# LuchnikovI/Differentiable-quantum-circuit-cuda

Hardware: AMD Instinct MI355X
Metric: gate-applications/sec (fwd+bwd) at n qubits (higher is better)
Workload: dtype c64 (f32)

## Files before the change

differentiable-quantum-circuit-cuda_amd/csrc/qdc.hip:

```cpp
#include "qdc_circuit.hpp"
#include "qdc_primitives.hpp"
#include "qdc_spec.hpp"

namespace {
template <int R>
struct SpecCheckTwo {
  __device__ __forceinline__ void operator()(qdc::cx (&xf)[R], qdc::cx (&xb)[R], const qdc::SpecEnv& E) const {
    constexpr uint32_t z[32] = {};
    qdc::spec_xchg_imm<6, false>(xf, E, z, z);
    qdc::spec_xchg<6, false>(xb, E, z, z, z, z);
  }
};
template <int R, int TB>
struct SpecCheckOne {
  __device__ __forceinline__ void operator()(qdc::cx (&x)[R], const qdc::SpecEnv& E) const {
    constexpr uint32_t z[32] = {};
    qdc::spec_xchg_imm<TB, true>(x, E, z, z);
    qdc::spec_xchg<TB, true>(x, E, z, z, z, z);
  }
};
}
#define QDC_SPEC_CHECK(name, threads, pass)                                                       \
  __global__ __launch_bounds__(threads) void name(qdc::chunk* f, qdc::chunk* b, const qdc::fop* ops, \
                                                  const qdc::cx* mats, qdc::fgeo fg, uint32_t l0,    \
// ... 381 lines not shown
#endif
}

QDC_API size_t qdc_fusion_schedule(size_t local_qubits, int backward, size_t first_inject,
                                   const int* kinds, const unsigned char* inexact,
                                   size_t n_instr, const qdc_plan_op* plan, size_t n_plan,
                                   int lcmin, int max_ops, unsigned* item_info, size_t item_cap,
                                   unsigned* stage_len, size_t stage_cap, unsigned* op_order,
                                   size_t op_cap) {
  std::vector<qdc::Instr> ins(n_instr);
  for (size_t k = 0; k < n_instr; ++k) ins[k] = qdc::Instr{kinds[k], 0, 0};
  std::vector<uint8_t> sens(n_instr, 0);
  if (inexact)
    for (size_t k = 0; k < n_instr; ++k) sens[k] = inexact[k] ? 1 : 0;
  qdc::FusionPlanner P{ins, sens, (uint32_t)local_qubits, true, true,
                             max_ops > 0 ? (uint32_t)std::min(max_ops, qdc::FMAX_OPS)
                                         : (uint32_t)qdc::FMAX_OPS,
                             lcmin > 0 ? (uint32_t)lcmin : 3u};
  using qdc::Knob;
  P.tile2_chunks = qdc::knob_uint(Knob::TILE2_CHUNKS, P.tile2_chunks);
  P.tile1_chunks = qdc::knob_uint(Knob::TILE1_CHUNKS, P.tile1_chunks);
  P.permute = P.rq_grad = qdc::knob_int(Knob::SCHED_RQ, 0) != 0;
  P.permute = qdc::knob_int(Knob::SCHED_PERM, P.permute) != 0;
  P.mirror = qdc::knob_int(Knob::SCHED_MIRROR, P.mirror) != 0;
  P.defer_q1 = qdc::knob_int(Knob::DEFER_Q1, P.defer_q1) != 0;
  P.search = qdc::knob_int(Knob::FUSE_SEARCH, P.search) != 0;
  P.perm_low = qdc::knob_uint(Knob::RQ_PERM_LOW, P.perm_low);
  P.gamma_stage_cap = qdc::knob_int(Knob::RQ_GSTAGE, P.gamma_stage_cap) != 0;
  P.split_dens = qdc::knob_int(Knob::DENS_SPLIT, P.split_dens) != 0;
  std::vector<qdc_plan_op> pl(plan, plan + n_plan);
  const std::vector<qdc::FusionItem> items = P.fuse_items(pl, backward != 0, first_inject);
  size_t ns = 0, no = 0;
  for (size_t i = 0; i < items.size(); ++i) {
    const qdc::FusionItem& it = items[i];
    std::vector<std::vector<uint32_t>> stages;
    if (it.type == qdc::ITEM_FUSED)
      stages = P.stage_partition(it.ops, pl, backward != 0);
    else
      stages.push_back(it.ops);
// ... 344 lines not shown
```

differentiable-quantum-circuit-cuda_amd/csrc/qdc_circuit.hpp:

```cpp
#pragma once

#include <algorithm>
#include <cstring>
#include <memory>
#include <vector>

#include <rccl/rccl.h>

#include "qdc/circuit.h"
#include "qdc_device.hpp"
#include "qdc_shard.hpp"
#include "qdc_stage.hpp"
#include "qdc_fusion.hpp"
#include "qdc_spec.hpp"

namespace qdc {

struct Flat {
  const qdc_complex* data;
  std::vector<size_t> off;
  std::vector<size_t> len;
  Flat(const qdc_complex* d, const size_t* lens, size_t n) : data(d), off(n), len(n) {
    size_t o = 0;
    for (size_t i = 0; i < n; ++i) {
// ... 151 lines not shown
  uint32_t n = 0;
  uint32_t g = 0;
  uint32_t nl = 0;
  uint32_t gap_bits = 0;
  uint64_t gm = 0;
  std::vector<std::unique_ptr<DevRes>> devs;
  Exchange ex;
  std::vector<Shard> sh;
  QubitMap layout;
  size_t dens_cap = 0, grads_cap = 0;
  cx* host_out = nullptr;
  size_t host_cap = 0;
  std::vector<Instr> ins;
  struct Knobs {
    int fuse = 1;
    uint32_t fuse_max_ops = FMAX_OPS;
    uint32_t fuse_lcmin = 3;
    int fuse_meas = 1;
    int use_rq = 1;
    int rq_stats = 0;
    RqKnobs rqk;
    int rq64 = 1;
    int rq_order = 2;
    int spec_mode = 1;
    uint32_t spec_min_qubits = 22;
    uint32_t spec_max = 160;
    int spec_fwd = 1;
    int spec_async = sizeof(real) == 4 ? 1 : 0;
    int rq_permute = 1;
    int rq_perm_shard = 1;
    int rq_grad32 = 1;
    int rq_maxcl = 1;
    uint32_t rq_perm_low = 0;
    int rq_gstage = 1;
    uint32_t tile1_chunks = FusionPlanner::TILE_CHUNKS_1;
    int diag_inject = 1;
    int early_inject = 1;
    int dens1_kernel = 1;
    int dens_split = 1;
    int mirror = 1;
    int spec_half = 1;
    int defer_q1 = 1;
    int fuse_search = 1;
    uint32_t fused_blocks = 0;
    int sched_cache_on = 1;
    int state_ilv = 1;
// ... 5 lines not shown
      f(Knob::FUSE_MAX_OPS, k.fuse_max_ops, 1, FMAX_OPS);
      f(Knob::FUSE_MEAS, k.fuse_meas);
      f(Knob::FUSE_LCMIN, k.fuse_lcmin, 1, LOWBITS);
      f(Knob::FUSED_BLOCKS, k.fused_blocks, 1, (int)NBMAX);
      f(Knob::RQ, k.use_rq);
      f(Knob::RQ64, k.rq64);
      f(Knob::RQ_STATS, k.rq_stats);
      f(Knob::RW, k.rqk.rq_wave);
      f(Knob::RQ_PF, k.rqk.rq_prefetch);
      f(Knob::RQ_SLOTS5, k.rqk.rq_slots5);
      f(Knob::RQ_ORDER, k.rq_order);
      f(Knob::RQ_PERM, k.rq_permute);
      f(Knob::RQ_PERM_SHARD, k.rq_perm_shard);
      f(Knob::RQ_PERM_LOW, k.rq_perm_low);
      f(Knob::RQ_GRAD32, k.rq_grad32);
      f(Knob::RQ_MAXCL, k.rq_maxcl);
      f(Knob::RQ_GSTAGE, k.rq_gstage);
      f(Knob::TILE1_CHUNKS, k.tile1_chunks);
      f(Knob::DIAG_INJECT, k.diag_inject);
      f(Knob::EARLY_INJECT, k.early_inject);
      f(Knob::DENS1, k.dens1_kernel);
      f(Knob::DENS_SPLIT, k.dens_split);
      f(Knob::MIRROR, k.mirror);
      f(Knob::DEFER_Q1, k.defer_q1);
      f(Knob::FUSE_SEARCH, k.fuse_search);
      f(Knob::SCHED_CACHE, k.sched_cache_on);
      f(Knob::SPEC, k.spec_mode);
      f(Knob::SPEC_MIN_QUBITS, k.spec_min_qubits);
      f(Knob::SPEC_MAX, k.spec_max);
      f(Knob::SPEC_FWD, k.spec_fwd);
// ... 522 lines not shown
    c.first_inject = first_injection(pl);
    return true;
  }
  size_t first_injection(const std::vector<qdc_plan_op>& pl) const {
    for (size_t i = 0; i < pl.size(); ++i)
      if (pl[i].type == QDC_PLAN_OP && is_diff_density(ins[pl[i].instr].kind)) return i;
    return pl.size();
  }
  static constexpr uint32_t TILE_CHUNKS_1 = FusionPlanner::TILE_CHUNKS_1;
  static constexpr uint32_t TILE_CHUNKS_2 = FusionPlanner::TILE_CHUNKS_2;
  FusionPlanner planner(bool mirror_fwd) const {
    FusionPlanner P{ins, inexact, nl, k.fuse != 0, k.fuse_meas != 0, k.fuse_max_ops, k.fuse_lcmin};
    P.permute = k.rq_permute && k.use_rq && (g == 0 || k.rq_perm_shard) && sizeof(real) == 4;
    P.ng = g;
    P.rq_grad = k.rq_grad32 && k.use_rq && (sizeof(real) == 4 || k.rq64);
    if (k.rq_perm_low) P.perm_low = k.rq_perm_low;
    P.tile1_chunks = k.tile1_chunks;
    P.mirror = mirror_on() && mirror_fwd;
    P.defer_q1 = k.defer_q1 != 0;
    P.search = k.fuse_search != 0;
    P.gamma_stage_cap = k.rq_gstage != 0;
    P.split_dens = k.dens_split != 0;
    return P;
  }
  void fuse_items(Call& c) const {
    c.items.clear();
    for (FusionItem& f : c.P.fuse_items(c.plan, c.backward, c.first_inject)) {
      Item it;
      static_cast<FusionItem&>(it) = std::move(f);
      if (it.type == ITEM_FUSED) it.stages = c.P.stage_partition(it.ops, c.plan, c.backward);
// ... 553 lines not shown
    auto kern = k_dens1<TB, NT>;
    QDC_TRY(fused_grid((const void*)kern, nullptr, NT, use.grid));
    fgeo g = fg;
    QDC_TRY(size_grid(ctx, g, use, false, "density"));
    return ctx.launch_block(name, bytes, kern, use.grid, (uint32_t)NT, (const chunk*)f, fops, g,
                            partials, stride);
  }
  const char* launch_rq(Ctx& ctx, const char* name, double bytes, const fgeo& fg, bool two,
                        uint32_t tbits, const RqVariant* V, uint32_t l0, chunk* f, chunk* b,
                        const fop* fops, const cx* mats, cx* partials, uint64_t stride,
                        hipFunction_t spec, GridUse& use) {
    if (!V || V->two != two || V->tbits != tbits || (spec && !V->prefix))
      return fail("internal: a register-resident pass without its kernel variant");
    if (!two && fg.ngrad > 0)
      return fail("internal: a one-state register-resident pass with %u reductions", fg.ngrad);
    QDC_TRY(fused_grid((const void*)V->kernel, spec && V->own_grid ? spec : nullptr, (int)V->threads,
                       use.grid));
    fgeo g = fg;
    QDC_TRY(size_grid(ctx, g, use, V->dyn, "fused"));
    if (spec)
      return ctx.launch_module(name, bytes, spec, use.grid, V->threads, f, b, fops, mats, g, l0,
                               partials, stride);
    return ctx.launch_block(name, bytes, V->kernel, use.grid, V->threads, f, b, fops, mats, g, l0,
                            partials, stride);
  }
  const char* fused_grid(const void* kernel, hipFunction_t fn, int nt, uint32_t& grid) {
    if (k.fused_blocks) {
      grid = k.fused_blocks;
      return nullptr;
    }
    const void* key = fn ? (const void*)fn : kernel;
    for (auto& e : fused_resident_cache)
      if (e.first == key) {
        grid = e.second;
        return nullptr;
      }
    int per_cu = 0, dev = 0, cus = 0;
    if (fn)
// ... 409 lines not shown
```

differentiable-quantum-circuit-cuda_amd/csrc/qdc_fusion.hpp:

```cpp
#pragma once

#include <stdint.h>

#include <algorithm>
#include <vector>

#include "qdc/circuit.h"
#include "qdc_kernels.hpp"
#include "qdc_knobs.hpp"
#include "qdc_rq.hpp"
#include "qdc_shard.hpp"

namespace qdc {

struct Instr {
  int kind;
  uint32_t a;
  uint32_t b;
};

inline bool is_q1_gate(int k) {
  return k == QDC_CONST_Q1 || k == QDC_CONST_Q1_NONU || k == QDC_VAR_Q1 || k == QDC_VAR_Q1_NONU;
}
inline bool is_q2_dense(int k) {
// ... 22 lines not shown
inline bool is_q1_density(int k) { return k == QDC_Q1_DENSITY || k == QDC_DIFF_Q1_DENSITY; }
inline int gate_len(int k) { return is_q2_dense(k) ? 16 : 4; }

enum ItemType : int {
  ITEM_OP = 0,
  ITEM_REMAP = 1,
  ITEM_FUSED = 2,
  ITEM_DIAG_INJECT = 3,
};
struct FusionItem {
  int type;
  std::vector<uint32_t> ops;
  uint32_t lc = 0, h = 0, hb[FMAX_ROWS] = {};
  std::vector<std::pair<uint32_t, uint32_t>> swaps;
};

struct FusionPlanner {
  static constexpr uint32_t TILE_CHUNKS_1 = 2048;
  static constexpr uint32_t TILE_CHUNKS_2 = 1024;
  const std::vector<Instr>& ins;
  const std::vector<uint8_t>& inexact;
  uint32_t nl;
  bool fuse;
  bool fuse_meas;
  uint32_t fuse_max_ops;
  uint32_t fuse_lcmin;
  uint32_t tile2_chunks = TILE_CHUNKS_2;
  uint32_t tile1_chunks = TILE_CHUNKS_1;
  bool permute = false;
  bool rq_grad = false;
  bool gamma_stage_cap = true;
  uint32_t perm_low = (uint32_t)LV + 3;
  uint32_t ng = 0;
  bool mirror = false;
  bool defer_q1 = true;
  bool split_dens = true;
  bool search = true;

  static uint32_t log2_of(uint64_t x) {
    uint32_t k = 0;
    while ((1ull << k) < x) ++k;
    return k;
  }

  uint64_t chunk_bits_of(uint32_t p) const { return p >= (uint32_t)LV ? 1ull << (p - LV) : 0ull; }
// ... 159 lines not shown
        ++i;
        continue;
      }
      if (!on || !fusable(i)) {
        items.push_back(FusionItem{ITEM_OP, {(uint32_t)i}});
        ++i;
        continue;
      }
      size_t j = i;
      while (j < plan.size() && plan[j].type == QDC_PLAN_OP && fusable(j) &&
             !(backward && j == first_inject && j > i) && !(j == msplit && j > i))
        ++j;
      const bool two = (backward && i >= first_inject) || mfwd;
      const bool gstage = two && rq_grad && gamma_stage_cap;
      const uint32_t gmax = gstage ? fuse_max_ops
                            : (two && rq_grad) ? (uint32_t)FMAX_GRAD_RQ : (uint32_t)FMAX_GRAD;
      const PassRules rules{backward, mfwd, two, gstage, gmax, T};
      std::vector<uint32_t> rem;
      for (size_t k = i; k < j; ++k) rem.push_back((uint32_t)k);
      while (!rem.empty()) {
        ScannedPass sp = search ? search_pass(plan, rem, rules)
                                : scan_pass(plan, rem.data(), rem.size(), rules, ~0ull, false);
        if (sp.ops.size() == 1) {
          items.push_back(FusionItem{ITEM_OP, sp.ops});
        } else {
          FusionItem it{ITEM_FUSED, sp.ops};
          tile_config(sp.mask, T, it.lc, it.h, it.hb);
          bool gates_only = it.lc >= NLOW - LV;
          for (uint32_t k : sp.ops) gates_only = gates_only && is_gate_op(plan[k]);
          if (permute && gates_only) permute_after(it, plan, sp.rest, j);
          items.push_back(it);
// ... 42 lines not shown
          (q & blocked) ||
          (mfwd && meas && ndens + 1 > (uint32_t)FMAX_GRAD) ||
          (conflicts_of(cls) & left) || pass.size() >= fuse_max_ops ||
          nred + isred > r.gmax || !tile_fits(mask | op_bits(g), r.T)) {
        blocked |= q;
        left |= cls;
        rest.push_back(k);
        continue;
      }
      pass.push_back(k);
      mask |= op_bits(g);
      nred += isred;
      ndens += (mfwd && meas) ? 1u : 0u;
      kind = (int)meas;
    }
    if (r.gstage && nred > (uint32_t)FMAX_GRAD_RQ) {
      bool cut = false;
      while (pass.size() > 1 && gamma_stages(pass, plan, !mfwd) > (uint32_t)FMAX_GRAD_RQ) {
        rest.push_back(pass.back());
        pass.pop_back();
        cut = true;
      }
      if (cut) std::sort(rest.begin(), rest.end());
    }
    if (defer_q1) defer_trailing_q1(pass, rest, plan, backward, per_qubit);
    for (uint32_t k : pass) sp.mask |= op_bits(plan[k]);
    return sp;
  }

  static constexpr size_t SEARCH_SEEDS = 8;
  static constexpr size_t SEARCH_WINDOW = 512;

  uint64_t tile_positions(uint64_t pos, uint32_t T) const {
// ... 1 lines not shown
    if (!tile_config(pos >> LV, T, lc, h, hb)) return 0;
    uint64_t a = (1ull << (LV + lc)) - 1;
    for (uint32_t r = 0; r < h; ++r) a |= 1ull << (LV + hb[r]);
    return a;
  }
  static uint64_t pos_bits(const qdc_plan_op& g) { return (1ull << g.pos2) | (1ull << g.pos1); }

  ScannedPass search_pass(const std::vector<qdc_plan_op>& plan, const std::vector<uint32_t>& rem,
                          const PassRules& r) const {
    ScannedPass base = scan_pass(plan, rem.data(), rem.size(), r, ~0ull, false);
    const size_t nw = std::min(rem.size(), SEARCH_WINDOW);
    auto stages_of = [&](const ScannedPass& p) {
      return (uint32_t)stage_partition(p.ops, plan, r.backward).size();
    };
    auto at_cap = [&](const ScannedPass& p, uint32_t st) {
      return p.ops.size() >= fuse_max_ops || (r.gstage && st >= (uint32_t)FMAX_GRAD_RQ) ||
             p.rest.empty();
    };
    auto width = [&](const ScannedPass& p) {
      uint64_t q = (1ull << NLOW) - 1;
      for (uint32_t k : p.ops) q |= pos_bits(plan[k]);
      return (uint32_t)__builtin_popcountll(q);
    };
    const uint32_t base_st = stages_of(base);
    if (at_cap(base, base_st) || nw < 3) return base;

    struct Cand {
      uint64_t tile;
      ScannedPass p;
      uint32_t st;
    };
// ... 482 lines not shown
```

differentiable-quantum-circuit-cuda_amd/csrc/qdc_jit.hpp:

```cpp
#pragma once

#include <dirent.h>
#include <dlfcn.h>
#include <fcntl.h>
#include <spawn.h>
#include <sys/file.h>
#include <sys/stat.h>
#include <sys/wait.h>
#include <unistd.h>

#include <algorithm>
#include <atomic>
#include <chrono>
#include <cerrno>
#include <condition_variable>
#include <csignal>
#include <cstdlib>
#include <deque>
#include <ctime>
#include <cstdio>
#include <cstring>
#include <map>
#include <mutex>
#include <set>
// ... 16 lines not shown

inline bool spec_imm() {
  static const bool on = knob_int(Knob::SPEC_IMM, 0) != 0;
  return on;
}
struct SpecStep {
  bool relayout;
  RqLayout Lc, Ln;
  fop F;
};
struct SpecKind {
  bool two;
  uint32_t tb, ns;
  bool bar;
  const char* prefix;
  const char* pass;
  uint32_t threads;
  const char* waves;
  bool half = false;
};
inline SpecKind spec_kind(const RqVariant& V, bool half = false) {
  uint32_t tb = 0;
  while ((1u << tb) < V.threads) ++tb;
  return {V.two, tb, V.ns, V.threads > 64, V.prefix, half ? V.pass_half : V.pass, V.threads,
          half ? V.waves_half : V.waves, half};
}
inline int spec_kept_slot(const RqLayout& Lc, const RqLayout& Ln) {
  if (Lc.ns != Ln.ns) return -1;
  for (uint32_t s = 0; s < Lc.ns; ++s)
    if (Lc.slot[s] == Ln.slot[s] && Lc.slot[s] != ~0u) return (int)s;
  return -1;
}
inline bool spec_half_ok(const std::vector<SpecStep>& steps) {
  bool any = false;
  for (const SpecStep& s : steps)
    if (s.relayout) {
      any = true;
      if (spec_kept_slot(s.Lc, s.Ln) < 0) return false;
    }
  return any;
// ... 191 lines not shown
           (int)QDC_RW_WAVES, (int)QDC_RW_WAVES_ONE, (int)QDC_RQ_ABL, (int)QDC_RQ_GSPLIT,
           (int)QDC_NT_LOAD, (int)QDC_NT_STORE, (int)QDC_RW_WAVES_HALF_ONE, (int)QDC_PK_ASM, (int)QDC_PK_VASM, (int)QDC_MATVEC_N,
           sizeof(real) == 8 ? " -DQDC_F64" : "");
  return b;
}
inline const char* spec_cflags() { return "--genco -O3 -std=c++17 --offload-arch=gfx950"; }
inline uint64_t spec_fingerprint(const std::string& defines, const std::string& compiler,
                                 uint64_t source_fp) {
  uint64_t h = 1469598103934665603ull;
  const std::string s = defines + "\n" + compiler + "\n" + spec_cflags() + "\n";
  h = fnv_more(h, s.data(), s.size());
  return fnv_more(h, &source_fp, sizeof source_fp);
}
inline std::string spec_kernel_name_fp(const std::string& body, const SpecKind& K, uint64_t fp) {
  char nm[48];
  uint64_t h = spec_hash(std::string(K.pass) + "\n" + body);
  h = fnv_more(h, &fp, sizeof fp);
  snprintf(nm, sizeof nm, "%s%016llx", K.prefix, (unsigned long long)h);
  return nm;
}

#ifndef QDC_SRC_FP
#define QDC_SRC_FP 0ull
#endif

struct JitObjHeader {
  char magic[8];
  uint64_t fp, name_hash, size, body_hash;
};
static_assert(sizeof(JitObjHeader) == 40, "code-object header layout");
constexpr char JIT_MAGIC[8] = {'Q', 'D', 'C', 'J', 'I', 'T', '2', '\0'};
// ... 577 lines not shown
```

differentiable-quantum-circuit-cuda_amd/csrc/qdc_kernels.hpp:

```cpp
#pragma once

#include <cstddef>

#include <hip/hip_runtime.h>
#include <stdint.h>

#include <type_traits>

namespace qdc {

#ifdef QDC_F64
using real = double;
typedef double vec16 __attribute__((ext_vector_type(2)));
#else
using real = float;
typedef float vec16 __attribute__((ext_vector_type(4)));
#endif

struct cx {
  real x, y;
};

constexpr int VEC = 16 / (int)sizeof(cx);
constexpr int LV = (VEC == 2) ? 1 : 0;
// ... 881 lines not shown
#pragma unroll
    for (int k = 0; k < RED; ++k) acc[k] = cadd(acc[k], q[k]);
  }
  __shared__ cx out[RED];
  block_reduce_store<RED>(acc, out);
  __syncthreads();
  if (threadIdx.x < RED) {
    cx* d = tab.dst[blockIdx.x] + threadIdx.x;
    *d = accumulate ? cadd(*d, out[threadIdx.x]) : out[threadIdx.x];
  }
}
#endif


#ifndef QDC_FMAX_OPS
#define QDC_FMAX_OPS 32
#endif
constexpr int FMAX_OPS = QDC_FMAX_OPS;
constexpr int FMAX_GRAD = 16;
#ifndef QDC_FMAX_GRAD_RQ
#define QDC_FMAX_GRAD_RQ 16
#endif
constexpr int FMAX_GRAD_RQ = QDC_FMAX_GRAD_RQ;
static_assert(FMAX_GRAD_RQ >= 1 && FMAX_GRAD >= 1, "at least one reduction accumulator");
static_assert(FMAX_OPS <= 64, "rq_plan keeps stage sets in 64-bit masks");
constexpr int FMAX_ROWS = 8;
constexpr int FACC = 32;

struct fop {
  uint32_t kind;
  uint32_t t1;
  uint32_t t2;
  uint32_t mat;
};

struct fgeo {
  uint64_t ntiles;
  uint32_t tpb;
  uint32_t lc;
// ... 854 lines not shown
```

differentiable-quantum-circuit-cuda_amd/csrc/qdc_knobs.hpp:

```cpp
#pragma once

#include <stdint.h>

#include <algorithm>
#include <climits>
#include <cstdio>
#include <cstdlib>
#include <string>

namespace qdc {

enum class KnobScope { Process, Context, Circuit, Call, Hook };

#define QDC_KNOBS(X)                                                                               \
                                                        \
  X(DYN, Context, "35",                                                                            \
    "static share (% of the fair share) of a dynamic-tail pass; 100: static only")                 \
  X(DYN_GRAN, Context, "1",                                                                        \
    "smallest granule (tiles per grab, a power of two <= 32) of a reducing dynamic tail")          \
  X(EVENT_FENCE, Context, "0",                                                                     \
    "1: the profiler's HIP events are default events (system-scope fence per record)")             \
  X(GRID_CAP, Context, "1048576", "grid cap of the single-gate streaming kernels")                 \
  X(RED_CAP, Context, "2048", "grid of the single-gate reduction kernels (<= 4096)")               \
  X(REV_RED, Context, "4096",                                                                      \
// ... 12 lines not shown
  X(DIAG_RU, Context, "16",                                                                        \
    "chunks per state in flight per thread of the diagonal reverse kernels")                       \
  X(DIAG_Q, Context, "1", "0: diagonal reverse launches on k_diag instead of k_diag_q")            \
  X(DIAG_RED, Context, "4096", "grid of the diagonal reverse's reducing launches (<= 4096)")       \
  X(TILE_PF, Context, "1", "0: tile-family blocks of several tiles do not prefetch the next tile") \
  X(LANE_BLK, Context, "1",                                                                        \
    "0: far-target streaming LANE launches stay on the wave variant, not k_lane_blk")              \
  X(LANE_TILE_BITS, Context, "0x8800000",                                                          \
    "mask of target byte strides 2^b whose one-state q1 applications run on the tile family")      \
  X(LANE_NOBLK_BITS, Context, "0x808000",                                                          \
    "mask of target byte strides 2^b whose far LANE applications run on the wave variant")         \
  X(LANE_U, Context, "8,1,4",                                                                      \
    "units in flight per wave of LANE launches, \"u0,u1,u2\" per op class as QDC_LANE")            \
                                                   \
  X(FUSE, Circuit, "1", "0: one HBM pass per gate (single-gate kernels only)")                     \
  X(FUSE_MAX_OPS, Circuit, "32", "gates per fused pass (1 .. FMAX_OPS)")                           \
  X(FUSE_MEAS, Circuit, "1", "0: densities / cotangent injections stay single passes")             \
  X(FUSE_LCMIN, Circuit, "3", "minimum contiguous chunk bits of a fused tile (1 .. 6)")            \
  X(FUSED_BLOCKS, Circuit, "0",                                                                    \
    "grid of fused passes (1 .. 4096); 0: as many blocks as are resident")                         \
  X(RQ, Circuit, "1", "0: gate passes on the LDS-tile kernel, not the register-resident ones")     \
  X(RQ64, Circuit, "1", "0: f64 gate passes stay on the LDS-tile kernel")                          \
  X(RQ_STATS, Circuit, "0",                                                                        \
    "1: print each register-resident pass's counts to stderr; 2: its stages too")                  \
  X(RW, Circuit, "1", "register-resident kernel choice, a bit mask (qdc_variant.hpp)")             \
  X(RQ_PF, Circuit, "1", "0: one-state register-resident passes do not prefetch the next tile")    \
  X(RQ_SLOTS5, Circuit, "1", "0: f32 one-wave passes plan four register slots, not five")          \
  X(RQ_ORDER, Circuit, "2",                                                                        \
    "register-resident tile order: 0 block-contiguous, 1 grid-strided, 2 XCD-aware")               \
  X(RQ_PERM, Circuit, "1", "0: gate-only passes keep the qubit layout (no in-store permutation)")  \
  X(RQ_PERM_SHARD, Circuit, "1", "0: no permuting passes on sharded circuits")                     \
  X(RQ_PERM_LOW, Circuit, "0", "low positions a permuting pass fills; 0: the planner's default")   \
  X(RQ_GRAD32, Circuit, "1",                                                                       \
    "0: two-state passes hold FMAX_GRAD instead of FMAX_GRAD_RQ Gamma stages")                     \
  X(RQ_MAXCL, Circuit, "1", "0: relayouts chosen greedily instead of by max closure")              \
  X(RQ_GSTAGE, Circuit, "1",                                                                       \
    "0: two-state passes capped by variable gates instead of Gamma stages")                        \
  X(TILE1_CHUNKS, Circuit, "2048", "one-state fused tile in chunks: 2048 or 1024")                 \
  X(DIAG_INJECT, Circuit, "1",                                                                     \
    "0: runs of diagonal cotangent injections stay fused injection passes")                        \
  X(EARLY_INJECT, Circuit, "1",                                                                    \
    "0: the backward's leading diagonal injection waits for its program")                          \
  X(DENS1, Circuit, "1", "0: read-only one-qubit density passes on k_fused instead of k_dens1")    \
  X(DENS_SPLIT, Circuit, "1", "0: a forward pass may hold gates and densities together")           \
  X(MIRROR, Circuit, "1",                                                                          \
    "mirrored reverse sweeps; 0: the backward schedules itself; 2: failing to mirror is an "       \
    "error")                                                                                       \
  X(DEFER_Q1, Circuit, "1", "0: trailing one-qubit stages of a pass stay there")                   \
  X(FUSE_SEARCH, Circuit, "1",                                                                     \
// ... 30 lines not shown
  X(QK_WIDE, Call, "k >= 4: 1, else 0",                                                            \
    "dense k-qubit kernel: doubled batches per wave iteration")                                    \
  X(QK_PF, Call, "k = 3: 2, k = 5: 1, else 0",                                                     \
    "dense k-qubit kernel: 1 software-pipelined batches, 2 doubled too")                           \
  X(QK_GRID, Call, "4096", "block cap of the dense k-qubit kernels' grids")                        \
  X(QK_LDS, Call, "k = 3: 2, else 1",                                                              \
    "low targets from which a dense gate runs as LDS-staged tiles; 0: never")                      \
  X(QKL_VAR, Call, "1", "k_qkl variant: 0 not pipelined, 1 pipelined, 2 half the tiles at k = 5")  \
  X(QKG_GRID, Call, "resident blocks", "block cap of the dense gradient / density kernel")         \
  X(PAULI_GRID, Call, "per kernel", "block cap of the Pauli-sum kernels")                          \
                                                     \
  X(SCHED_RQ, Hook, "0",                                                                           \
    "qdc_fusion_schedule: permuting passes and the register-resident Gamma cap")                   \
  X(SCHED_PERM, Hook, "as QDC_SCHED_RQ", "qdc_fusion_schedule: permuting passes alone")            \
  X(SCHED_MIRROR, Hook, "0", "qdc_fusion_schedule: the mirrored forward schedule")                 \
  X(TILE2_CHUNKS, Hook, "1024", "qdc_fusion_schedule: two-state fused tile in chunks")             \
  X(RQ_KEEP, Hook, "0", "qdc_rq_plan: every relayout keeps a register slot (half buffers)")        \
  X(PRECOMPILE_DUMP, Hook, "unset",                                                                \
    "qdc_precompile: directory that receives each kernel's source")                                \
  X(PRECOMPILE_COUNT, Hook, "0", "qdc_precompile: 1 counts the kernels without compiling them")

enum class Knob : int {
#define QDC_KNOB_ID(id, scope, dflt, effect) id,
  QDC_KNOBS(QDC_KNOB_ID)
#undef QDC_KNOB_ID
};

struct KnobRow {
  const char* name;
  KnobScope scope;
// ... 72 lines not shown
```

differentiable-quantum-circuit-cuda_amd/csrc/qdc_rq.hpp:

```cpp
#pragma once

#include <type_traits>

#include "qdc_kernels.hpp"

namespace qdc {

#ifndef QDC_RQ_GSPLIT
#define QDC_RQ_GSPLIT 0
#endif
#ifndef QDC_MATVEC_N
#define QDC_MATVEC_N 1
#endif

constexpr int RQ_R = 16;
constexpr uint32_t FK_RELAYOUT = 7;
constexpr int RQ_NT_ONE = 256;
constexpr int RQ_NT_TWO = 128;

struct rq_layout {
  uint32_t rp[2 * RQ_R];
  uint32_t tv[8];
};
static_assert(sizeof(rq_layout) == 160 && sizeof(rq_layout) % sizeof(cx) == 0,
// ... 358 lines not shown
               : "+{a[64:67]}"(v[16]), "+{a[68:71]}"(v[17]), "+{a[72:75]}"(v[18]), "+{a[76:79]}"(v[19]), "+{a[80:83]}"(v[20]), "+{a[84:87]}"(v[21]), "+{a[88:91]}"(v[22]), "+{a[92:95]}"(v[23]), "+{a[96:99]}"(v[24]), "+{a[100:103]}"(v[25]), "+{a[104:107]}"(v[26]), "+{a[108:111]}"(v[27]), "+{a[112:115]}"(v[28]), "+{a[116:119]}"(v[29]), "+{a[120:123]}"(v[30]), "+{a[124:127]}"(v[31])
               :
               : "memory");
}

#ifndef QDC_RQ_PF_WAVES
#define QDC_RQ_PF_WAVES 2
#endif
struct SpecEnv {
  const cx* mats;
  const fop* ops;
  real (*accw)[FACC];
  uint32_t t;
  char* bufb;
};
template <bool TWO, int NT, bool PF, class PROG = void>
__device__ __forceinline__ void rq_pass(chunk* __restrict__ f, chunk* __restrict__ b,
                                        const fop* __restrict__ ops, const cx* __restrict__ mats,
                                        fgeo fg, uint32_t l0, cx* __restrict__ partials,
                                        uint64_t slot_stride) {
  constexpr int LOGNT = NT == 64 ? 6 : NT == 128 ? 7 : NT == 256 ? 8 : 9;
  constexpr int CPT = RQ_R / VEC;
  constexpr int TA = NT * RQ_R;
  __shared__ cx buf[TA];
  __shared__ real accw[TWO ? NT / 64 : 1][TWO ? FMAX_GRAD_RQ : 1][FACC];
  const uint32_t t = threadIdx.x;
  const int wave = __builtin_amdgcn_readfirstlane((int)(t >> 6));
  if constexpr (TWO) {
    for (uint32_t i = t; i < (NT / 64) * FMAX_GRAD_RQ * FACC; i += NT) (&accw[0][0][0])[i] = 0;
    __syncthreads();
  }
  const rq_layout* L0 = reinterpret_cast<const rq_layout*>(mats + l0);
  const rqio* io = reinterpret_cast<const rqio*>(mats + l0 + sizeof(rq_layout) / sizeof(cx));
  uint64_t thr_ld = 0, thr_st = 0;
#pragma unroll
  for (int k = 0; k < LOGNT; ++k) {
    if ((t >> k) & 1u) {
      thr_ld += io->gv_ld[k];
      thr_st += io->gv_st[k];
    }
  }
  const bool gstride = fg.order == 1;
  const uint64_t tile0 = gstride ? (uint64_t)blockIdx.x
                                 : (uint64_t)xcd_block(blockIdx.x, gridDim.x, fg.order == 2) * fg.tpb;
// ... 167 lines not shown
      }
      if (!more) break;
    }
  }
  if constexpr (TWO) {
    __syncthreads();
    for (uint32_t i = t; i < fg.ngrad * FACC; i += NT) {
      const uint32_t k = i / FACC, e = i % FACC;
      real s = 0;
#pragma unroll
      for (int w = 0; w < NT / 64; ++w) s += accw[w][k][e];
      reinterpret_cast<real*>(partials + (uint64_t)k * slot_stride + (uint64_t)blockIdx.x * RED)[e] = s;
    }
  }
}
template <bool TWO, int NT, bool PF>
__global__ __launch_bounds__(NT) __attribute__((amdgpu_waves_per_eu(PF ? QDC_RQ_PF_WAVES : 4)))
void k_rq(chunk* __restrict__ f, chunk* __restrict__ b, const fop* __restrict__ ops,
          const cx* __restrict__ mats, fgeo fg, uint32_t l0, cx* __restrict__ partials,
          uint64_t slot_stride) {
  static_assert(TWO ? (NT == 128 && !PF) : (NT == 128 || NT == 256), "k_rq: not a launched variant");
  rq_pass<TWO, NT, PF>(f, b, ops, mats, fg, l0, partials, slot_stride);
}

#ifndef QDC_RW_WAVES
#define QDC_RW_WAVES 2
#endif
#ifndef QDC_RW_WAVES_HALF_ONE
#define QDC_RW_WAVES_HALF_ONE 5
#endif
#ifndef QDC_RW_WAVES_ONE
#define QDC_RW_WAVES_ONE 2
#endif
template <bool TWO, int NE, bool PF, int W, bool S5 = false, class PROG = void, bool HALF = false>
__device__ __forceinline__ void rw_pass(chunk* __restrict__ f, chunk* __restrict__ b,
                                        const fop* __restrict__ ops, const cx* __restrict__ mats,
                                        fgeo fg, uint32_t l0, cx* __restrict__ partials,
                                        uint64_t slot_stride) {
  static_assert(NE == 1 || NE == 2 || NE == 4, "k_rw: 1, 2 or 4 register groups");
  static_assert(!S5 || (NE == 2 && VEC == 2 && W == 1 && (!PF || !TWO)),
                "five slots: f32 one-wave tiles (two-state ones without prefetch)");
  static_assert(W == 1 || (W == 2 && !TWO), "k_rw: two-state tiles are one wave");
  constexpr int LOGNE = NE == 1 ? 0 : NE == 2 ? 1 : 2;
  constexpr int TB = W == 1 ? 6 : 7;
  constexpr int R = RQ_R * NE;
  constexpr int CPT = R / VEC;
  constexpr int CPG = RQ_R / VEC;
  static_assert(!HALF || (W == 1 && !std::is_void<PROG>::value), "half buffers: one-wave programs");
  __shared__ cx buf[64 * W * R / (HALF ? 2 : 1)];
  __shared__ real accw[TWO ? FMAX_GRAD_RQ : 1][FACC];
  const uint32_t lane = threadIdx.x;
  if constexpr (TWO) {
    for (uint32_t i = lane; i < FMAX_GRAD_RQ * FACC; i += 64) (&accw[0][0])[i] = 0;
  }
  const rqio* io = reinterpret_cast<const rqio*>(mats + l0 + sizeof(rq_layout) / sizeof(cx));
  uint64_t thr_ld = 0, thr_st = 0;
#pragma unroll
  for (int k = 0; k < TB; ++k) {
    if ((lane >> k) & 1u) {
      thr_ld += io->gv_ld[k];
      thr_st += io->gv_st[k];
    }
  }
  const bool gstride = fg.order == 1;
  const uint64_t tile0 = gstride ? (uint64_t)blockIdx.x
                                 : (uint64_t)xcd_block(blockIdx.x, gridDim.x, fg.order == 2) * fg.tpb;
  const uint64_t tstep = gstride ? (uint64_t)gridDim.x : 1u;
  const uint64_t nst = (QDC_DYN_TAIL && fg_arg()->ndyn) ? fg_arg()->nstat : fg.ntiles;
// ... 304 lines not shown
        store(xf, xb, prev);
      }
    }
  }
  if constexpr (TWO) {
    if (PF || W != 1 || !QDC_DYN_TAIL || !fg_arg()->ndyn) {
      __builtin_amdgcn_wave_barrier();
      for (uint32_t i = lane; i < fg.ngrad * FACC; i += 64) {
        const uint32_t k = i / FACC, e = i % FACC;
        reinterpret_cast<real*>(partials + (uint64_t)k * slot_stride + (uint64_t)blockIdx.x * RED)[e] =
            accw[k][e];
      }
    }
  }
}
template <bool TWO, int NE, bool PF, int W, bool S5 = false>
__global__ __launch_bounds__(64 * W) __attribute__((amdgpu_waves_per_eu(
    (PF && TWO) ? 1 : (!TWO && !PF) ? QDC_RW_WAVES_ONE : QDC_RW_WAVES,
    (PF && TWO) ? 1 : (!TWO && !PF) ? QDC_RW_WAVES_ONE : QDC_RW_WAVES)))
void k_rw(chunk* __restrict__ f, chunk* __restrict__ b, const fop* __restrict__ ops,
          const cx* __restrict__ mats, fgeo fg, uint32_t l0, cx* __restrict__ partials,
          uint64_t slot_stride) {
  static_assert(NE == 2 ? (VEC == 2 && (TWO ? (W == 1 && !(PF && S5))
                                            : (W == 1 ? (!PF || S5) : (W == 2 && !PF && !S5))))
                        : (NE == 1 && VEC == 1 && !PF && !S5 && (W == 1 || (W == 2 && !TWO))),
                "k_rw: not a launched variant");
  rw_pass<TWO, NE, PF, W, S5>(f, b, ops, mats, fg, l0, partials, slot_stride);
}

}
```

differentiable-quantum-circuit-cuda_amd/csrc/qdc_spec.hpp:

```cpp
#pragma once

#include "qdc_rq.hpp"

namespace qdc {

template <int TB, bool BAR, int R>
__device__ __forceinline__ void spec_xchg(cx (&x)[R], const SpecEnv& E, const uint32_t* rpc,
                                          const uint32_t* tvc, const uint32_t* rpn,
                                          const uint32_t* tvn) {
  uint32_t tp = 0, tpn = 0;
#pragma unroll
  for (int k = 0; k < TB; ++k) {
    tp ^= ((E.t >> k) & 1u) ? tvc[k] : 0u;
    tpn ^= ((E.t >> k) & 1u) ? tvn[k] : 0u;
  }
  uint32_t tpb = tp * (uint32_t)sizeof(cx), tpnb = tpn * (uint32_t)sizeof(cx);
  asm volatile("" : "+v"(tpb), "+v"(tpnb));
  if constexpr (BAR) __syncthreads();
#pragma unroll
  for (int j = 0; j < R; ++j)
    *reinterpret_cast<cx*>(__builtin_assume_aligned(E.bufb + (tpb ^ (rpc[j] * (uint32_t)sizeof(cx))), 8)) = x[j];
  if constexpr (BAR)
    __syncthreads();
  else
// ... 56 lines not shown
  if constexpr (!BAR) __builtin_amdgcn_wave_barrier();
}

}

#ifndef QDC_SPEC_TU
#include "qdc_jit.hpp"

namespace qdc {

inline bool spec_half_buffer(const RqVariant& V, bool spec_half, const std::vector<SpecStep>& steps) {
  return V.pass_half && spec_half && !spec_imm() && spec_half_ok(steps);
}
inline SpecEntry spec_kernel_of(const std::vector<SpecStep>& steps, const RqVariant& V,
                                uint32_t tbits, bool half) {
  const SpecKind K = spec_kind(V, half);
  const std::string body = spec_program_source(steps, tbits, K);
  SpecEntry e;
  e.name = spec_kernel_name(body, K);
  e.src = spec_kernel_source(e.name, body, K);
  return e;
}

}
#endif
```

differentiable-quantum-circuit-cuda_amd/csrc/qdc_variant.hpp:

```cpp
#pragma once

#include "qdc_rq.hpp"

namespace qdc {

using rq_kernel_t = void (*)(chunk*, chunk*, const fop*, const cx*, fgeo, uint32_t, cx*, uint64_t);

struct RqVariant {
  const char* label;
  rq_kernel_t kernel;
  bool two;
  uint32_t tbits;
  uint32_t threads;
  uint32_t ns;
  bool dyn;
  const char* prefix;
  const char* pass;
  const char* waves;
  const char* pass_half;
  const char* waves_half;
  bool own_grid;
};

#define QDC_RQ_KERNEL(...) #__VA_ARGS__, __VA_ARGS__
#define QDC_RQ_NO_SPEC nullptr, nullptr, nullptr, nullptr, nullptr, false
#ifndef QDC_F64
enum RqVariantId {
  RV_TWO_S5, RV_TWO, RV_TWO_AGPR, RV_TWO_RQ,
  RV_ONE_S5, RV_ONE_S5_PF, RV_ONE, RV_ONE_RQ_PF, RV_ONE_RQ,
  RV_ONE12_RW, RV_ONE12_RQ_PF, RV_ONE12_RQ,
  RV_COUNT
};
inline const RqVariant* rq_variants() {
  static const RqVariant V[RV_COUNT] = {
      {QDC_RQ_KERNEL(k_rw<true, 2, false, 1, true>), true, 11, 64, 5, true, "qdc_spec_",
       "qdc::rw_pass<true, 2, false, 1, true, Prog>", "QDC_RW_WAVES, QDC_RW_WAVES",
       "qdc::rw_pass<true, 2, false, 1, true, Prog, true>", "QDC_RW_WAVES, QDC_RW_WAVES", true},
      {QDC_RQ_KERNEL(k_rw<true, 2, false, 1>), true, 11, 64, 4, true, QDC_RQ_NO_SPEC},
      {QDC_RQ_KERNEL(k_rw<true, 2, true, 1>), true, 11, 64, 4, false, QDC_RQ_NO_SPEC},
      {QDC_RQ_KERNEL(k_rq<true, 128, false>), true, 11, 128, 4, false, QDC_RQ_NO_SPEC},
      {QDC_RQ_KERNEL(k_rw<false, 2, false, 1, true>), false, 11, 64, 5, true, "qdc_specf_",
       "qdc::rw_pass<false, 2, false, 1, true, Prog>", "QDC_RW_WAVES_ONE, QDC_RW_WAVES_ONE",
       "qdc::rw_pass<false, 2, false, 1, true, Prog, true>",
       "QDC_RW_WAVES_HALF_ONE, QDC_RW_WAVES_HALF_ONE", true},
      {QDC_RQ_KERNEL(k_rw<false, 2, true, 1, true>), false, 11, 64, 5, true, "qdc_specf_",
       "qdc::rw_pass<false, 2, true, 1, true, Prog>", "QDC_RW_WAVES, QDC_RW_WAVES", nullptr, nullptr,
       false},
      {QDC_RQ_KERNEL(k_rw<false, 2, false, 1>), false, 11, 64, 4, true, QDC_RQ_NO_SPEC},
      {QDC_RQ_KERNEL(k_rq<false, 128, true>), false, 11, 128, 4, true, QDC_RQ_NO_SPEC},
      {QDC_RQ_KERNEL(k_rq<false, 128, false>), false, 11, 128, 4, false, QDC_RQ_NO_SPEC},
      {QDC_RQ_KERNEL(k_rw<false, 2, false, 2>), false, 12, 128, 4, false, QDC_RQ_NO_SPEC},
      {QDC_RQ_KERNEL(k_rq<false, 256, true>), false, 12, 256, 4, true, "qdc_specf_",
       "qdc::rq_pass<false, 256, true, Prog>", "QDC_RQ_PF_WAVES", nullptr, nullptr, false},
      {QDC_RQ_KERNEL(k_rq<false, 256, false>), false, 12, 256, 4, false, QDC_RQ_NO_SPEC},
  };
  return V;
}
#else
enum RqVariantId { RV_TWO, RV_ONE, RV_ONE11, RV_COUNT };
inline const RqVariant* rq_variants() {
  static const RqVariant V[RV_COUNT] = {
      {QDC_RQ_KERNEL(k_rw<true, 1, false, 1>), true, 10, 64, 4, true, "qdc_spec_d_",
       "qdc::rw_pass<true, 1, false, 1, false, Prog>", "QDC_RW_WAVES, QDC_RW_WAVES", nullptr, nullptr,
       false},
      {QDC_RQ_KERNEL(k_rw<false, 1, false, 1>), false, 10, 64, 4, true, "qdc_specf_d_",
       "qdc::rw_pass<false, 1, false, 1, false, Prog>", "QDC_RW_WAVES_ONE, QDC_RW_WAVES_ONE", nullptr,
       nullptr, false},
      {QDC_RQ_KERNEL(k_rw<false, 1, false, 2>), false, 11, 128, 4, false, "qdc_specf_d_",
       "qdc::rw_pass<false, 1, false, 2, false, Prog>", "QDC_RW_WAVES_ONE, QDC_RW_WAVES_ONE", nullptr,
       nullptr, false},
  };
  return V;
}
#endif
#undef QDC_RQ_KERNEL
#undef QDC_RQ_NO_SPEC

struct RqKnobs {
  int rq_wave = 1;
// ... 35 lines not shown
```

Baseline: 5262.

## Fuse more gates and Gamma stages per pass with wide-accumulator kernel variants

Doubles the compile-time fusion caps (ops per fused pass to 64, Gamma stages per two-state register pass to 32 in f32) and adds a runtime gamma_cap knob the planner uses. A second instantiation of each two-state kernel with a larger shared accumulator array is chosen when a pass holds more than 16 Gamma stages, and the JIT spec path emits the wider template argument to match. The aim is fewer HBM passes over the state vector in forward and backward. In exchange, the wide kernels use more LDS per block, which may lower occupancy, and longer fused programs raise register pressure and compile cost.

Result: faster. 5524, median of 6 (+5.0%).

```diff
diff --git a/differentiable-quantum-circuit-cuda_amd/csrc/qdc.hip b/differentiable-quantum-circuit-cuda_amd/csrc/qdc.hip
--- a/differentiable-quantum-circuit-cuda_amd/csrc/qdc.hip
+++ b/differentiable-quantum-circuit-cuda_amd/csrc/qdc.hip
@@ -419,8 +419,7 @@
   if (inexact)
     for (size_t k = 0; k < n_instr; ++k) sens[k] = inexact[k] ? 1 : 0;
   qdc::FusionPlanner P{ins, sens, (uint32_t)local_qubits, true, true,
-                             max_ops > 0 ? (uint32_t)std::min(max_ops, qdc::FMAX_OPS)
-                                         : (uint32_t)qdc::FMAX_OPS,
+                             max_ops > 0 ? (uint32_t)std::min(max_ops, qdc::FMAX_OPS) : 32u,
                              lcmin > 0 ? (uint32_t)lcmin : 3u};
   using qdc::Knob;
   P.tile2_chunks = qdc::knob_uint(Knob::TILE2_CHUNKS, P.tile2_chunks);
@@ -428,6 +427,7 @@
   P.permute = P.rq_grad = qdc::knob_int(Knob::SCHED_RQ, 0) != 0;
   P.permute = qdc::knob_int(Knob::SCHED_PERM, P.permute) != 0;
   P.mirror = qdc::knob_int(Knob::SCHED_MIRROR, P.mirror) != 0;
+  P.gamma_cap = (uint32_t)qdc::knob_int(Knob::SCHED_GCAP, 16, 1, qdc::FMAX_GRAD_RQ);
   P.defer_q1 = qdc::knob_int(Knob::DEFER_Q1, P.defer_q1) != 0;
   P.search = qdc::knob_int(Knob::FUSE_SEARCH, P.search) != 0;
   P.perm_low = qdc::knob_uint(Knob::RQ_PERM_LOW, P.perm_low);
diff --git a/differentiable-quantum-circuit-cuda_amd/csrc/qdc_circuit.hpp b/differentiable-quantum-circuit-cuda_amd/csrc/qdc_circuit.hpp
--- a/differentiable-quantum-circuit-cuda_amd/csrc/qdc_circuit.hpp
+++ b/differentiable-quantum-circuit-cuda_amd/csrc/qdc_circuit.hpp
@@ -189,7 +189,7 @@
   std::vector<Instr> ins;
   struct Knobs {
     int fuse = 1;
-    uint32_t fuse_max_ops = FMAX_OPS;
+    uint32_t fuse_max_ops = 2 * RQ_GCAP_DEFAULT;
     uint32_t fuse_lcmin = 3;
     int fuse_meas = 1;
     int use_rq = 1;
@@ -205,6 +205,7 @@
     int rq_permute = 1;
     int rq_perm_shard = 1;
     int rq_grad32 = 1;
+    uint32_t rq_gcap = RQ_GCAP_DEFAULT;
     int rq_maxcl = 1;
     uint32_t rq_perm_low = 0;
     int rq_gstage = 1;
@@ -240,6 +241,7 @@
       f(Knob::RQ_PERM_SHARD, k.rq_perm_shard);
       f(Knob::RQ_PERM_LOW, k.rq_perm_low);
       f(Knob::RQ_GRAD32, k.rq_grad32);
+      f(Knob::RQ_GCAP, k.rq_gcap, 1, FMAX_GRAD_RQ);
       f(Knob::RQ_MAXCL, k.rq_maxcl);
       f(Knob::RQ_GSTAGE, k.rq_gstage);
       f(Knob::TILE1_CHUNKS, k.tile1_chunks);
@@ -792,6 +794,7 @@
     P.permute = k.rq_permute && k.use_rq && (g == 0 || k.rq_perm_shard) && sizeof(real) == 4;
     P.ng = g;
     P.rq_grad = k.rq_grad32 && k.use_rq && (sizeof(real) == 4 || k.rq64);
+    P.gamma_cap = k.rq_gcap;
     if (k.rq_perm_low) P.perm_low = k.rq_perm_low;
     P.tile1_chunks = k.tile1_chunks;
     P.mirror = mirror_on() && mirror_fwd;
@@ -1375,14 +1378,15 @@
       return fail("internal: a register-resident pass without its kernel variant");
     if (!two && fg.ngrad > 0)
       return fail("internal: a one-state register-resident pass with %u reductions", fg.ngrad);
-    QDC_TRY(fused_grid((const void*)V->kernel, spec && V->own_grid ? spec : nullptr, (int)V->threads,
+    const rq_kernel_t kernel = V->kernel_for(fg.ngrad);
+    QDC_TRY(fused_grid((const void*)kernel, spec && V->own_grid ? spec : nullptr, (int)V->threads,
                        use.grid));
     fgeo g = fg;
     QDC_TRY(size_grid(ctx, g, use, V->dyn, "fused"));
     if (spec)
       return ctx.launch_module(name, bytes, spec, use.grid, V->threads, f, b, fops, mats, g, l0,
                                partials, stride);
-    return ctx.launch_block(name, bytes, V->kernel, use.grid, V->threads, f, b, fops, mats, g, l0,
+    return ctx.launch_block(name, bytes, kernel, use.grid, V->threads, f, b, fops, mats, g, l0,
                             partials, stride);
   }
   const char* fused_grid(const void* kernel, hipFunction_t fn, int nt, uint32_t& grid) {
diff --git a/differentiable-quantum-circuit-cuda_amd/csrc/qdc_fusion.hpp b/differentiable-quantum-circuit-cuda_amd/csrc/qdc_fusion.hpp
--- a/differentiable-quantum-circuit-cuda_amd/csrc/qdc_fusion.hpp
+++ b/differentiable-quantum-circuit-cuda_amd/csrc/qdc_fusion.hpp
@@ -60,6 +60,10 @@
   uint32_t lc = 0, h = 0, hb[FMAX_ROWS] = {};
   std::vector<std::pair<uint32_t, uint32_t>> swaps;
 };
+
+constexpr uint32_t RQ_GCAP_DEFAULT = sizeof(real) == 4 ? 32u : 16u;
+static_assert(RQ_GCAP_DEFAULT <= (uint32_t)FMAX_GRAD_RQ && 2 * RQ_GCAP_DEFAULT <= (uint32_t)FMAX_OPS,
+              "the default caps lie within the storage bounds");
 
 struct FusionPlanner {
   static constexpr uint32_t TILE_CHUNKS_1 = 2048;
@@ -75,6 +79,7 @@
   uint32_t tile1_chunks = TILE_CHUNKS_1;
   bool permute = false;
   bool rq_grad = false;
+  uint32_t gamma_cap = RQ_GCAP_DEFAULT;
   bool gamma_stage_cap = true;
   uint32_t perm_low = (uint32_t)LV + 3;
   uint32_t ng = 0;
@@ -264,7 +269,7 @@
       const bool two = (backward && i >= first_inject) || mfwd;
       const bool gstage = two && rq_grad && gamma_stage_cap;
       const uint32_t gmax = gstage ? fuse_max_ops
-                            : (two && rq_grad) ? (uint32_t)FMAX_GRAD_RQ : (uint32_t)FMAX_GRAD;
+                            : (two && rq_grad) ? gamma_cap : (uint32_t)FMAX_GRAD;
       const PassRules rules{backward, mfwd, two, gstage, gmax, T};
       std::vector<uint32_t> rem;
       for (size_t k = i; k < j; ++k) rem.push_back((uint32_t)k);
@@ -337,9 +342,9 @@
       ndens += (mfwd && meas) ? 1u : 0u;
       kind = (int)meas;
     }
-    if (r.gstage && nred > (uint32_t)FMAX_GRAD_RQ) {
+    if (r.gstage && nred > gamma_cap) {
       bool cut = false;
-      while (pass.size() > 1 && gamma_stages(pass, plan, !mfwd) > (uint32_t)FMAX_GRAD_RQ) {
+      while (pass.size() > 1 && gamma_stages(pass, plan, !mfwd) > gamma_cap) {
         rest.push_back(pass.back());
         pass.pop_back();
         cut = true;
@@ -371,7 +376,7 @@
       return (uint32_t)stage_partition(p.ops, plan, r.backward).size();
     };
     auto at_cap = [&](const ScannedPass& p, uint32_t st) {
-      return p.ops.size() >= fuse_max_ops || (r.gstage && st >= (uint32_t)FMAX_GRAD_RQ) ||
+      return p.ops.size() >= fuse_max_ops || (r.gstage && st >= gamma_cap) ||
              p.rest.empty();
     };
     auto width = [&](const ScannedPass& p) {
diff --git a/differentiable-quantum-circuit-cuda_amd/csrc/qdc_jit.hpp b/differentiable-quantum-circuit-cuda_amd/csrc/qdc_jit.hpp
--- a/differentiable-quantum-circuit-cuda_amd/csrc/qdc_jit.hpp
+++ b/differentiable-quantum-circuit-cuda_amd/csrc/qdc_jit.hpp
@@ -54,16 +54,26 @@
   uint32_t tb, ns;
   bool bar;
   const char* prefix;
-  const char* pass;
+  std::string pass;
   uint32_t threads;
   const char* waves;
   bool half = false;
 };
-inline SpecKind spec_kind(const RqVariant& V, bool half = false) {
+inline SpecKind spec_kind(const RqVariant& V, bool half = false, uint32_t gamma = 0) {
   uint32_t tb = 0;
   while ((1u << tb) < V.threads) ++tb;
-  return {V.two, tb, V.ns, V.threads > 64, V.prefix, half ? V.pass_half : V.pass, V.threads,
+  std::string pass = half ? V.pass_half : V.pass;
+  if (V.two && gamma > (uint32_t)RQ_GACC_SMALL) {
+    pass.pop_back();
+    pass += std::string(half ? "" : ", false") + ", " + std::to_string((int)FMAX_GRAD_RQ) + ">";
+  }
+  return {V.two, tb, V.ns, V.threads > 64, V.prefix, pass, V.threads,
           half ? V.waves_half : V.waves, half};
+}
+inline uint32_t spec_gamma_stages(const std::vector<SpecStep>& steps) {
+  uint32_t n = 0;
+  for (const SpecStep& s : steps) n += (!s.relayout && (s.F.kind & FOP_GAMMA)) ? 1u : 0u;
+  return n;
 }
 inline int spec_kept_slot(const RqLayout& Lc, const RqLayout& Ln) {
   if (Lc.ns != Ln.ns) return -1;
@@ -285,7 +295,7 @@
 }
 inline std::string spec_kernel_name_fp(const std::string& body, const SpecKind& K, uint64_t fp) {
   char nm[48];
-  uint64_t h = spec_hash(std::string(K.pass) + "\n" + body);
+  uint64_t h = spec_hash(K.pass + "\n" + body);
   h = fnv_more(h, &fp, sizeof fp);
   snprintf(nm, sizeof nm, "%s%016llx", K.prefix, (unsigned long long)h);
   return nm;
diff --git a/differentiable-quantum-circuit-cuda_amd/csrc/qdc_kernels.hpp b/differentiable-quantum-circuit-cuda_amd/csrc/qdc_kernels.hpp
--- a/differentiable-quantum-circuit-cuda_amd/csrc/qdc_kernels.hpp
+++ b/differentiable-quantum-circuit-cuda_amd/csrc/qdc_kernels.hpp
@@ -919,15 +919,17 @@
 
 
 #ifndef QDC_FMAX_OPS
-#define QDC_FMAX_OPS 32
+#define QDC_FMAX_OPS 64
 #endif
 constexpr int FMAX_OPS = QDC_FMAX_OPS;
 constexpr int FMAX_GRAD = 16;
 #ifndef QDC_FMAX_GRAD_RQ
-#define QDC_FMAX_GRAD_RQ 16
+#define QDC_FMAX_GRAD_RQ 32
 #endif
 constexpr int FMAX_GRAD_RQ = QDC_FMAX_GRAD_RQ;
+constexpr int RQ_GACC_SMALL = FMAX_GRAD_RQ < 16 ? FMAX_GRAD_RQ : 16;
 static_assert(FMAX_GRAD_RQ >= 1 && FMAX_GRAD >= 1, "at least one reduction accumulator");
+static_assert(FMAX_GRAD_RQ <= FIN_MAX, "a pass's partial slots are pending together (Ctx::flush)");
 static_assert(FMAX_OPS <= 64, "rq_plan keeps stage sets in 64-bit masks");
 constexpr int FMAX_ROWS = 8;
 constexpr int FACC = 32;
diff --git a/differentiable-quantum-circuit-cuda_amd/csrc/qdc_knobs.hpp b/differentiable-quantum-circuit-cuda_amd/csrc/qdc_knobs.hpp
--- a/differentiable-quantum-circuit-cuda_amd/csrc/qdc_knobs.hpp
+++ b/differentiable-quantum-circuit-cuda_amd/csrc/qdc_knobs.hpp
@@ -50,7 +50,7 @@
     "units in flight per wave of LANE launches, \"u0,u1,u2\" per op class as QDC_LANE")            \
                                                    \
   X(FUSE, Circuit, "1", "0: one HBM pass per gate (single-gate kernels only)")                     \
-  X(FUSE_MAX_OPS, Circuit, "32", "gates per fused pass (1 .. FMAX_OPS)")                           \
+  X(FUSE_MAX_OPS, Circuit, "f32: 64, f64: 32", "gates per fused pass (1 .. FMAX_OPS)")             \
   X(FUSE_MEAS, Circuit, "1", "0: densities / cotangent injections stay single passes")             \
   X(FUSE_LCMIN, Circuit, "3", "minimum contiguous chunk bits of a fused tile (1 .. 6)")            \
   X(FUSED_BLOCKS, Circuit, "0",                                                                    \
@@ -68,7 +68,9 @@
   X(RQ_PERM_SHARD, Circuit, "1", "0: no permuting passes on sharded circuits")                     \
   X(RQ_PERM_LOW, Circuit, "0", "low positions a permuting pass fills; 0: the planner's default")   \
   X(RQ_GRAD32, Circuit, "1",                                                                       \
-    "0: two-state passes hold FMAX_GRAD instead of FMAX_GRAD_RQ Gamma stages")                     \
+    "0: two-state passes hold FMAX_GRAD instead of QDC_RQ_GCAP Gamma stages")                      \
+  X(RQ_GCAP, Circuit, "f32: 32, f64: 16",                                                          \
+    "Gamma stages a two-state register-resident pass holds (1 .. FMAX_GRAD_RQ)")                   \
   X(RQ_MAXCL, Circuit, "1", "0: relayouts chosen greedily instead of by max closure")              \
   X(RQ_GSTAGE, Circuit, "1",                                                                       \
     "0: two-state passes capped by variable gates instead of Gamma stages")                        \
@@ -129,6 +131,8 @@
     "qdc_fusion_schedule: permuting passes and the register-resident Gamma cap")                   \
   X(SCHED_PERM, Hook, "as QDC_SCHED_RQ", "qdc_fusion_schedule: permuting passes alone")            \
   X(SCHED_MIRROR, Hook, "0", "qdc_fusion_schedule: the mirrored forward schedule")                 \
+  X(SCHED_GCAP, Hook, "16",                                                                        \
+    "qdc_fusion_schedule: Gamma stages of a two-state pass (1 .. FMAX_GRAD_RQ)")                   \
   X(TILE2_CHUNKS, Hook, "1024", "qdc_fusion_schedule: two-state fused tile in chunks")             \
   X(RQ_KEEP, Hook, "0", "qdc_rq_plan: every relayout keeps a register slot (half buffers)")        \
   X(PRECOMPILE_DUMP, Hook, "unset",                                                                \
diff --git a/differentiable-quantum-circuit-cuda_amd/csrc/qdc_rq.hpp b/differentiable-quantum-circuit-cuda_amd/csrc/qdc_rq.hpp
--- a/differentiable-quantum-circuit-cuda_amd/csrc/qdc_rq.hpp
+++ b/differentiable-quantum-circuit-cuda_amd/csrc/qdc_rq.hpp
@@ -396,7 +396,7 @@
   uint32_t t;
   char* bufb;
 };
-template <bool TWO, int NT, bool PF, class PROG = void>
+template <bool TWO, int NT, bool PF, class PROG = void, int GA = RQ_GACC_SMALL>
 __device__ __forceinline__ void rq_pass(chunk* __restrict__ f, chunk* __restrict__ b,
                                         const fop* __restrict__ ops, const cx* __restrict__ mats,
                                         fgeo fg, uint32_t l0, cx* __restrict__ partials,
@@ -405,11 +405,11 @@
   constexpr int CPT = RQ_R / VEC;
   constexpr int TA = NT * RQ_R;
   __shared__ cx buf[TA];
-  __shared__ real accw[TWO ? NT / 64 : 1][TWO ? FMAX_GRAD_RQ : 1][FACC];
+  __shared__ real accw[TWO ? NT / 64 : 1][TWO ? GA : 1][FACC];
   const uint32_t t = threadIdx.x;
   const int wave = __builtin_amdgcn_readfirstlane((int)(t >> 6));
   if constexpr (TWO) {
-    for (uint32_t i = t; i < (NT / 64) * FMAX_GRAD_RQ * FACC; i += NT) (&accw[0][0][0])[i] = 0;
+    for (uint32_t i = t; i < (NT / 64) * GA * FACC; i += NT) (&accw[0][0][0])[i] = 0;
     __syncthreads();
   }
   const rq_layout* L0 = reinterpret_cast<const rq_layout*>(mats + l0);
@@ -607,13 +607,14 @@
     }
   }
 }
-template <bool TWO, int NT, bool PF>
+template <bool TWO, int NT, bool PF, int GA = RQ_GACC_SMALL>
 __global__ __launch_bounds__(NT) __attribute__((amdgpu_waves_per_eu(PF ? QDC_RQ_PF_WAVES : 4)))
 void k_rq(chunk* __restrict__ f, chunk* __restrict__ b, const fop* __restrict__ ops,
           const cx* __restrict__ mats, fgeo fg, uint32_t l0, cx* __restrict__ partials,
           uint64_t slot_stride) {
   static_assert(TWO ? (NT == 128 && !PF) : (NT == 128 || NT == 256), "k_rq: not a launched variant");
-  rq_pass<TWO, NT, PF>(f, b, ops, mats, fg, l0, partials, slot_stride);
+  static_assert(TWO || GA == RQ_GACC_SMALL, "one-state passes hold no accumulators");
+  rq_pass<TWO, NT, PF, void, GA>(f, b, ops, mats, fg, l0, partials, slot_stride);
 }
 
 #ifndef QDC_RW_WAVES
@@ -625,7 +626,8 @@
 #ifndef QDC_RW_WAVES_ONE
 #define QDC_RW_WAVES_ONE 2
 #endif
-template <bool TWO, int NE, bool PF, int W, bool S5 = false, class PROG = void, bool HALF = false>
+template <bool TWO, int NE, bool PF, int W, bool S5 = false, class PROG = void, bool HALF = false,
+          int GA = RQ_GACC_SMALL>
 __device__ __forceinline__ void rw_pass(chunk* __restrict__ f, chunk* __restrict__ b,
                                         const fop* __restrict__ ops, const cx* __restrict__ mats,
                                         fgeo fg, uint32_t l0, cx* __restrict__ partials,
@@ -641,10 +643,10 @@
   constexpr int CPG = RQ_R / VEC;
   static_assert(!HALF || (W == 1 && !std::is_void<PROG>::value), "half buffers: one-wave programs");
   __shared__ cx buf[64 * W * R / (HALF ? 2 : 1)];
-  __shared__ real accw[TWO ? FMAX_GRAD_RQ : 1][FACC];
+  __shared__ real accw[TWO ? GA : 1][FACC];
   const uint32_t lane = threadIdx.x;
   if constexpr (TWO) {
-    for (uint32_t i = lane; i < FMAX_GRAD_RQ * FACC; i += 64) (&accw[0][0])[i] = 0;
+    for (uint32_t i = lane; i < GA * FACC; i += 64) (&accw[0][0])[i] = 0;
   }
   const rqio* io = reinterpret_cast<const rqio*>(mats + l0 + sizeof(rq_layout) / sizeof(cx));
   uint64_t thr_ld = 0, thr_st = 0;
@@ -979,7 +981,7 @@
     }
   }
 }
-template <bool TWO, int NE, bool PF, int W, bool S5 = false>
+template <bool TWO, int NE, bool PF, int W, bool S5 = false, int GA = RQ_GACC_SMALL>
 __global__ __launch_bounds__(64 * W) __attribute__((amdgpu_waves_per_eu(
     (PF && TWO) ? 1 : (!TWO && !PF) ? QDC_RW_WAVES_ONE : QDC_RW_WAVES,
     (PF && TWO) ? 1 : (!TWO && !PF) ? QDC_RW_WAVES_ONE : QDC_RW_WAVES)))
@@ -990,7 +992,8 @@
                                             : (W == 1 ? (!PF || S5) : (W == 2 && !PF && !S5))))
                         : (NE == 1 && VEC == 1 && !PF && !S5 && (W == 1 || (W == 2 && !TWO))),
                 "k_rw: not a launched variant");
-  rw_pass<TWO, NE, PF, W, S5>(f, b, ops, mats, fg, l0, partials, slot_stride);
-}
-
-}
+  static_assert(TWO || GA == RQ_GACC_SMALL, "one-state passes hold no accumulators");
+  rw_pass<TWO, NE, PF, W, S5, void, false, GA>(f, b, ops, mats, fg, l0, partials, slot_stride);
+}
+
+}
diff --git a/differentiable-quantum-circuit-cuda_amd/csrc/qdc_spec.hpp b/differentiable-quantum-circuit-cuda_amd/csrc/qdc_spec.hpp
--- a/differentiable-quantum-circuit-cuda_amd/csrc/qdc_spec.hpp
+++ b/differentiable-quantum-circuit-cuda_amd/csrc/qdc_spec.hpp
@@ -94,7 +94,7 @@
 }
 inline SpecEntry spec_kernel_of(const std::vector<SpecStep>& steps, const RqVariant& V,
                                 uint32_t tbits, bool half) {
-  const SpecKind K = spec_kind(V, half);
+  const SpecKind K = spec_kind(V, half, spec_gamma_stages(steps));
   const std::string body = spec_program_source(steps, tbits, K);
   SpecEntry e;
   e.name = spec_kernel_name(body, K);
diff --git a/differentiable-quantum-circuit-cuda_amd/csrc/qdc_variant.hpp b/differentiable-quantum-circuit-cuda_amd/csrc/qdc_variant.hpp
--- a/differentiable-quantum-circuit-cuda_amd/csrc/qdc_variant.hpp
+++ b/differentiable-quantum-circuit-cuda_amd/csrc/qdc_variant.hpp
@@ -20,6 +20,10 @@
   const char* pass_half;
   const char* waves_half;
   bool own_grid;
+  rq_kernel_t kernel_wide = nullptr;
+  rq_kernel_t kernel_for(uint32_t gamma) const {
+    return gamma > (uint32_t)RQ_GACC_SMALL && kernel_wide ? kernel_wide : kernel;
+  }
 };
 
 #define QDC_RQ_KERNEL(...) #__VA_ARGS__, __VA_ARGS__
@@ -35,10 +39,14 @@
   static const RqVariant V[RV_COUNT] = {
       {QDC_RQ_KERNEL(k_rw<true, 2, false, 1, true>), true, 11, 64, 5, true, "qdc_spec_",
        "qdc::rw_pass<true, 2, false, 1, true, Prog>", "QDC_RW_WAVES, QDC_RW_WAVES",
-       "qdc::rw_pass<true, 2, false, 1, true, Prog, true>", "QDC_RW_WAVES, QDC_RW_WAVES", true},
-      {QDC_RQ_KERNEL(k_rw<true, 2, false, 1>), true, 11, 64, 4, true, QDC_RQ_NO_SPEC},
-      {QDC_RQ_KERNEL(k_rw<true, 2, true, 1>), true, 11, 64, 4, false, QDC_RQ_NO_SPEC},
-      {QDC_RQ_KERNEL(k_rq<true, 128, false>), true, 11, 128, 4, false, QDC_RQ_NO_SPEC},
+       "qdc::rw_pass<true, 2, false, 1, true, Prog, true>", "QDC_RW_WAVES, QDC_RW_WAVES", true,
+       k_rw<true, 2, false, 1, true, FMAX_GRAD_RQ>},
+      {QDC_RQ_KERNEL(k_rw<true, 2, false, 1>), true, 11, 64, 4, true, QDC_RQ_NO_SPEC,
+       k_rw<true, 2, false, 1, false, FMAX_GRAD_RQ>},
+      {QDC_RQ_KERNEL(k_rw<true, 2, true, 1>), true, 11, 64, 4, false, QDC_RQ_NO_SPEC,
+       k_rw<true, 2, true, 1, false, FMAX_GRAD_RQ>},
+      {QDC_RQ_KERNEL(k_rq<true, 128, false>), true, 11, 128, 4, false, QDC_RQ_NO_SPEC,
+       k_rq<true, 128, false, FMAX_GRAD_RQ>},
       {QDC_RQ_KERNEL(k_rw<false, 2, false, 1, true>), false, 11, 64, 5, true, "qdc_specf_",
        "qdc::rw_pass<false, 2, false, 1, true, Prog>", "QDC_RW_WAVES_ONE, QDC_RW_WAVES_ONE",
        "qdc::rw_pass<false, 2, false, 1, true, Prog, true>",
@@ -62,7 +70,7 @@
   static const RqVariant V[RV_COUNT] = {
       {QDC_RQ_KERNEL(k_rw<true, 1, false, 1>), true, 10, 64, 4, true, "qdc_spec_d_",
        "qdc::rw_pass<true, 1, false, 1, false, Prog>", "QDC_RW_WAVES, QDC_RW_WAVES", nullptr, nullptr,
-       false},
+       false, k_rw<true, 1, false, 1, false, FMAX_GRAD_RQ>},
       {QDC_RQ_KERNEL(k_rw<false, 1, false, 1>), false, 10, 64, 4, true, "qdc_specf_d_",
        "qdc::rw_pass<false, 1, false, 1, false, Prog>", "QDC_RW_WAVES_ONE, QDC_RW_WAVES_ONE", nullptr,
        nullptr, false},
```
